# ETM-Code/eirgrid

Measured on AMD Instinct MI355X. Metric: 26-year episodes/sec, higher is better.
Workload: dtype f64

## Files before the change

eirgrid_amd/_native.py:

```python
from __future__ import annotations

import ctypes as C
import os

YEARS, N_ACTIONS, N_DEFICIT, N_COUNTS, N_TYPES = 26, 61, 15, 21, 15
GRID, CELLS, YEARLY_FIELDS = 51, 2601, 21
MAX_GENS, MAX_OFFSETS, RUN_CAP, DEF_CAP, ACT_CAP, ONCHIP_GENS = 4096, 4096, 4096, 4096, 4096, 512
TOPK_MAX = 64
STATS_LEN = 8 + 2 * YEARS * N_ACTIONS + YEARS * N_DEFICIT
CANDIDATE_BYTES = 8 + 8 + 32 + 4 * YEARS + 4 * YEARS + RUN_CAP + DEF_CAP
PACKET_BYTES = 8 * STATS_LEN + CANDIDATE_BYTES

EG_OK, EG_ERR_NO_DEVICE, EG_ERR_BAD_ARG, EG_ERR_HIP, EG_ERR_UNSUPPORTED, EG_ERR_NOMEM, EG_ERR_INTERNAL = 0, -1, -2, -3, -4, -5, -6
EG_EP_OK, EG_EP_OVERFLOW, EG_EP_NO_LOCATION, EG_EP_INTERNAL = 0, -1, -2, -3

LIB_PATH = os.environ.get("EIRGRID_LIB") or os.path.join(os.path.dirname(os.path.abspath(__file__)), "libeirgrid_hip.so")

_dp = C.POINTER(C.c_double)
_u8p = C.POINTER(C.c_uint8)
_u16p = C.POINTER(C.c_uint16)
_u32p = C.POINTER(C.c_uint32)
_i32p = C.POINTER(C.c_int32)
_u64p = C.POINTER(C.c_uint64)

# ... 20 lines not shown
class EgEpisodeOut(C.Structure):
    _fields_ = [("metrics", _dp), ("yearly", _dp), ("status", _i32p), ("n_run", _i32p), ("n_def", _i32p), ("n_act", _i32p),
                ("run_log", _u8p), ("def_log", _u8p), ("act_log", _u8p), ("n_gens", _i32p), ("gen_cell", _u16p),
                ("gen_pack", _u16p), ("n_offsets", _i32p), ("off_pack", _u16p), ("n_draws", _u64p), ("bytes_moved", _dp),
                ("n_chunks", _u32p)]


class EgPlanSet(C.Structure):
    _fields_ = [("n_plans", C.c_int32), ("best_count", _i32p), ("best_actions", _u8p), ("best_deficit_count", _i32p),
                ("best_deficit_actions", _u8p), ("best_actions_len", C.c_int64), ("best_deficit_actions_len", C.c_int64),
                ("names", C.POINTER(C.c_char_p))]


EXPORTS = [
    "eg_build_hash", "eg_last_error", "eg_device_count", "eg_create", "eg_destroy", "eg_rollout_batch", "eg_upload_snapshot",
    "eg_rollout_launch", "eg_rollout_launch_update", "eg_sync", "eg_last_batch_size", "eg_policy_hold", "eg_policy_rewind", "eg_replay_hoist", "eg_replay_hoist_stats", "eg_debug_hoist_stamps", "eg_fetch", "eg_timing_reset", "eg_timing_read", "eg_timing_read_grids", "eg_memory_report", "eg_update_stats", "eg_fetch_scores",
    "eg_fetch_episode_lists", "eg_fetch_record", "eg_fetch_best_run", "eg_best_result_track", "eg_fetch_best_result", "eg_evaluate_action_impact", "eg_place", "eg_find_suitable_location", "eg_debug_fill_lds", "eg_debug_occupy", "eg_policy_apply_reduced", "eg_policy_apply_packet", "eg_train_step",
    "eg_policy_push", "eg_device_rollout", "eg_device_apply", "eg_device_step", "eg_policy_pull",
    "eg_group_create", "eg_group_destroy", "eg_group_rank", "eg_group_push", "eg_group_step", "eg_group_pull", "eg_group_replay_hoist",
    "eg_group_best_result_track", "eg_group_fetch_best_result", "eg_top_k_track", "eg_fetch_top_k", "eg_rank_score",
    "eg_group_top_k_track", "eg_group_fetch_top_k", "eg_plans_validate", "eg_evaluate_plans", "eg_plans_load", "eg_plans_free",
    "eg_host_tables_create", "eg_host_tables_free", "eg_host_tables_f64", "eg_host_tables_i32",
    "eg_policy_new", "eg_policy_free", "eg_policy_snapshot_view", "eg_policy_get_tables", "eg_policy_set_tables",
    "eg_policy_get_scalar", "eg_policy_set_scalar", "eg_policy_get_list", "eg_policy_apply_episode", "eg_score_metrics",
    "eg_policy_save_json", "eg_policy_load_json", "eg_policy_append_weight_history", "eg_policy_export_improvement_csv", "eg_export_summary_csv", "eg_export_run_details",
]

_lib = None


def source_hash() -> str:
# ... 37 lines not shown
    L.eg_rollout_launch_update.restype = C.c_int32
    L.eg_rollout_launch_update.argtypes = [C.c_void_p, C.c_uint64, C.c_uint64, C.c_uint32, _u8p, C.c_void_p]
    L.eg_sync.restype = C.c_int32
    L.eg_sync.argtypes = [C.c_void_p]
    L.eg_last_batch_size.restype = C.c_uint32
    for f in (L.eg_policy_hold, L.eg_policy_rewind):
        f.restype = C.c_int32; f.argtypes = [C.c_void_p]
    L.eg_last_batch_size.argtypes = [C.c_void_p]
    if hasattr(L, "eg_replay_hoist") or not os.environ.get("EIRGRID_LIB"):
        L.eg_replay_hoist.restype = C.c_int32
        L.eg_replay_hoist.argtypes = [C.c_void_p, C.c_int32]
        L.eg_replay_hoist_stats.restype = C.c_int32
        L.eg_replay_hoist_stats.argtypes = [C.c_void_p, _u64p, _i32p]
        L.eg_debug_hoist_stamps.restype = C.c_int32
        L.eg_debug_hoist_stamps.argtypes = [C.c_void_p, _u64p]
    L.eg_fetch.restype = C.c_int32
    L.eg_fetch.argtypes = [C.c_void_p, C.POINTER(EgEpisodeOut)]
    L.eg_timing_reset.restype = C.c_int32
    L.eg_timing_reset.argtypes = [C.c_void_p]
    L.eg_timing_read.restype = C.c_int32
    L.eg_timing_read.argtypes = [C.c_void_p, _dp, _i32p]
    if hasattr(L, "eg_memory_report") or not os.environ.get("EIRGRID_LIB"):
        L.eg_memory_report.restype = C.c_int32
        L.eg_memory_report.argtypes = [C.c_void_p, _u64p, _u64p, _u64p]
    L.eg_timing_read_grids.restype = C.c_int32
    L.eg_timing_read_grids.argtypes = [C.c_void_p, _dp, _dp, _i32p]
    L.eg_update_stats.restype = C.c_int32
    L.eg_update_stats.argtypes = [C.c_void_p, C.c_void_p]
    L.eg_fetch_scores.restype = C.c_int32
    L.eg_fetch_scores.argtypes = [C.c_void_p, _dp]
# ... 123 lines not shown
```

eirgrid_amd/csrc/eg_api.cpp:

```cpp
#include <hip/hip_runtime.h>

#include <algorithm>
#include <cmath>
#include <cstring>
#include <map>
#include <mutex>
#include <cstdlib>
#include <string>
#include <vector>

#include "eg_internal.h"
#include "eg_policy_internal.h"
#define EG_RM static inline
#include "eg_reduced_math.h"

namespace eg {
namespace {
thread_local std::string g_error;
}
void set_error(const std::string& s) { g_error = s; }
}

using namespace eg;

// ... 56 lines not shown
  uint32_t push_iteration_count = 0;
  uint32_t push_failed = 0;
  uint32_t pulled_improvements = 0;
  uint8_t* d_packet = nullptr; uint8_t* h_packet = nullptr;
  uint32_t helper_max_episodes = 0;
  uint32_t heavy_slots_max = uint32_t((size_t(64) << 30) / (size_t(kRadiusClasses) * 2624 * sizeof(double)));
  uint32_t heavy_slots_wanted = 4096, launch_epoch = 0;
  bool heavy_slots_auto = true;
  bool hoist_on = false, hoist_supported = false;
  unsigned long long hoist_seq = 0;
  HoistInfo* d_hoist = nullptr; uint8_t* d_coop = nullptr;
  uint64_t hoist_batches = 0;
  int coop_force = 0;
  long long* d_stats_rep = nullptr;
  bool stats_rep_dirty = false;
  unsigned long long* d_solo = nullptr; uint32_t solo_cap = 0; unsigned long long solo_seq = 0;
  bool solo_on = true;
  uint8_t* d_eval_snap = nullptr;
  uint8_t* d_plans = nullptr; uint32_t plans_cap = 0;
  uint32_t* d_plan_index = nullptr; uint32_t plan_index_cap = 0;
};

namespace {

template <typename T>
void put(std::vector<uint8_t>& blob, size_t off, const std::vector<T>& v, size_t max_count) {
  const size_t n = v.size() < max_count ? v.size() : max_count;
  if (n) std::memcpy(blob.data() + off, v.data(), sizeof(T) * n);
}

void free_outputs(eg_ctx* c) {
// ... 25 lines not shown
        sum += ms;
      }
    for (int a = 0; a < 2; ++a)
      for (int b = 0; b < 2; ++b) {
        if (!(a ? lean : heavy) || !(b ? lean : heavy)) continue;
        EG_HIP(hipEventSynchronize(c->ev[i][2 * b + 1]));
        float ms = 0.f;
        EG_HIP(hipEventElapsedTime(&ms, c->ev[i][2 * a], c->ev[i][2 * b + 1]));
        if (ms > best) best = ms;
      }
    c->total_ms += double(best); c->grids_ms += double(sum); c->n_launches += 1; c->ring_pending -= 1;
  }
  return EG_OK;
}
int prepare_heavy(eg_ctx* c, uint32_t n_heavy, bool known_short) {
  constexpr size_t kSlotBytes = size_t(kRadiusClasses) * 2624 * sizeof(double), kTileBytes = size_t(kMaxVariants) * 64 * sizeof(double);
  if (known_short && !c->dev.heavy) n_heavy = 0;
  uint32_t want = c->heavy_slots_wanted;
  if (c->heavy_slots_auto && want > 0) {
    while (want < n_heavy && want < c->heavy_slots_max) want = want * 2u < c->heavy_slots_max ? want * 2u : c->heavy_slots_max;
  }
  if (want > 0 && n_heavy > 0 && (!c->dev.heavy || want > c->dev.heavy_slots)) {
    void* pool = nullptr;
    if (c->dev.heavy) {
      EG_HIP(hipDeviceSynchronize());
      for (auto it = c->allocs.begin(); it != c->allocs.end(); ++it) if (*it == c->dev.heavy) { c->allocs.erase(it); break; }
      (void)hipFree(c->dev.heavy);
      c->dev.heavy = nullptr; c->dev.heavy_slots = 0; c->dev.heavy_tiles = nullptr;
    }
    if (!c->dev.heavy_claim) {
      void* claim = nullptr;
      if (hipMalloc(&claim, 64) != hipSuccess) { (void)hipGetLastError(); c->heavy_slots_wanted = 0; want = 0; }
      else { EG_HIP(hipMemset(claim, 0xFF, 64)); c->allocs.push_back(claim); c->dev.heavy_claim = static_cast<unsigned*>(claim); }
    }
    while (want > 0 && hipMalloc(&pool, (kSlotBytes + kTileBytes) * want) != hipSuccess) {
      (void)hipGetLastError();
      pool = nullptr;
      want = want > 4096u ? want / 2u : 0u;
      c->heavy_slots_auto = false; c->heavy_slots_wanted = want;
    }
    if (pool) {
      c->allocs.push_back(pool); c->dev.heavy = static_cast<uint8_t*>(pool); c->dev.heavy_slots = want;
      c->dev.heavy_tiles = reinterpret_cast<double*>(static_cast<uint8_t*>(pool) + kSlotBytes * want);
    }
  }
  c->launch_epoch = (c->launch_epoch + 1u) & 0xFFFu;
  if (c->launch_epoch == 0xFFFu) c->launch_epoch = 0u;
  c->dev.heavy_epoch = c->launch_epoch;
  return EG_OK;
}
int topk_select(eg_ctx* c, uint32_t n, uint64_t first_index, int mode, bool use_score_list, const uint8_t* d_state, int k) {
  if (n > c->tk_cap) {
    if (c->d_tk_score) (void)hipFree(c->d_tk_score);
    if (c->d_tk_key) (void)hipFree(c->d_tk_key);
    if (c->d_tk_blocks) (void)hipFree(c->d_tk_blocks);
    c->d_tk_score = nullptr; c->d_tk_key = nullptr; c->d_tk_blocks = nullptr; c->tk_cap = 0;
    EG_HIP(hipMalloc((void**)&c->d_tk_score, sizeof(double) * n));
    EG_HIP(hipMalloc((void**)&c->d_tk_key, sizeof(unsigned long long) * n));
// ... 54 lines not shown
    if (plan.d_stats_rep != nullptr && c->stats_rep_dirty) {
      if (c->stream_heavy) EG_HIP(hipStreamSynchronize(c->stream_heavy));
      EG_HIP(hipMemsetAsync(c->d_stats_rep, 0, sizeof(long long) * size_t(kStatsReplicas) * EG_STATS_LEN, nullptr));
      c->stats_rep_dirty = false;
    }
  }
  if (plan.n_heavy > 0 && !plan.helper_waves && !plan.skip_long && !c->hoist_on) {
    if (c->solo_on) {
      if (plan.n_heavy > c->solo_cap) {
        if (c->d_solo) (void)hipFree(c->d_solo);
        c->d_solo = nullptr; c->solo_cap = 0;
        EG_HIP(hipMalloc((void**)&c->d_solo, sizeof(unsigned long long) * plan.n_heavy));
        EG_HIP(hipMemsetAsync(c->d_solo, 0, sizeof(unsigned long long) * plan.n_heavy, nullptr));
        c->solo_cap = plan.n_heavy;
      }
      plan.solo_seq = ++c->solo_seq; plan.d_solo = c->d_solo;
    }
  }
  if (c->hoist_on && plan.n_heavy > 0) {
    plan.hoist_seq = ++c->hoist_seq; plan.d_hoist = c->d_hoist; plan.coop_out = c->d_coop; plan.coop_force = c->coop_force;
    c->hoist_batches += 1;
  }
  if (split) {
    EG_HIP(hipEventRecord(c->ev_fork[slot], nullptr));
    EG_HIP(hipStreamWaitEvent(c->stream_heavy, c->ev_fork[slot], 0));
    if (list_long || plan.hoist_seq != 0ull) plan.go_event = c->ev_go[slot];
  }
  if (plan.d_stats_rep != nullptr) c->stats_rep_dirty = true;
  const int lr = launch_rollout(c->dev, c->snap, c->out, seed, first_index, n, d_mask, period, d_stats, plan);
  if (lr != 0) { set_error(std::string("k_rollout launch: ") + hipGetErrorString((hipError_t)lr)); return EG_ERR_HIP; }
  if (split) {
// ... 32 lines not shown
    if (rc != EG_OK) return rc;
    if (c->dev.heavy && chunk > c->dev.heavy_slots) chunk = c->dev.heavy_slots;
    RolloutPlan plan{};
    plan.plans = true; plan.helper_waves = helper;
    plan.n_short = first ? n_short : 0u;
    plan.n_heavy = plan.n_short + chunk; plan.n_lean = 0; plan.mode = 1u;
    plan.d_index = c->d_plan_index; plan.d_index_long = c->d_plan_index + n_short + done;
    if (chunk > 0 && !helper && c->solo_on) {
      if (chunk > c->solo_cap) {
        if (c->d_solo) (void)hipFree(c->d_solo);
        c->d_solo = nullptr; c->solo_cap = 0;
        EG_HIP(hipMalloc((void**)&c->d_solo, sizeof(unsigned long long) * chunk));
        EG_HIP(hipMemsetAsync(c->d_solo, 0, sizeof(unsigned long long) * chunk, nullptr));
        c->solo_cap = chunk;
      }
      plan.solo_seq = ++c->solo_seq; plan.d_solo = c->d_solo;
    }
    if (c->ring_pending == eg_ctx::kTimingRing) { rc = collect_timing(c, 1); if (rc != EG_OK) return rc; }
    const int slot = c->ring_head;
    for (int k = 0; k < 4; ++k) plan.ev[k] = c->ev[slot][k];
    const int lr = launch_rollout(c->dev, S, c->out, seed, first_index, n, nullptr, 1u, nullptr, plan);
    if (lr != 0) { set_error(std::string("k_rollout launch (plan batch): ") + hipGetErrorString((hipError_t)lr)); return EG_ERR_HIP; }
    c->ev_used[slot] = 1;
    c->ring_head = (c->ring_head + 1) % eg_ctx::kTimingRing; c->ring_pending += 1;
    done += chunk;
  }
  c->last_n = n; c->last_first = first_index;
  return EG_OK;
}

}
// ... 759 lines not shown
  EG_HIP(hipMemcpy(&word, c->d_hoist, sizeof(word), hipMemcpyDeviceToHost));
  if (batches_armed) *batches_armed = c->hoist_batches;
  static_assert(offsetof(HoistInfo, served_seq) == 0, "the served word comes first");
  if (last_batch_hoisted) *last_batch_hoisted = (c->hoist_seq != 0ull && word == c->hoist_seq) ? 1 : 0;
  return EG_OK;
}

int32_t eg_debug_hoist_stamps(eg_ctx* c, uint64_t stamps[8]) {
  if (!c || !stamps) return EG_ERR_BAD_ARG;
  EG_HIP(hipSetDevice(c->device));
  EG_HIP(hipDeviceSynchronize());
  EG_HIP(hipMemcpy(stamps, reinterpret_cast<const uint8_t*>(c->d_hoist) + offsetof(HoistInfo, stamps), 8 * sizeof(uint64_t), hipMemcpyDeviceToHost));
  return EG_OK;
}

int32_t eg_policy_hold(eg_ctx* c) {
  if (!c || !c->snap_valid) { set_error("eg_policy_hold: push a policy first"); return EG_ERR_BAD_ARG; }
  EG_HIP(hipSetDevice(c->device));
  if (!c->d_snap_held) EG_HIP(hipMalloc((void**)&c->d_snap_held, snap::total));
  EG_HIP(hipMemcpyAsync(c->d_snap_held, c->d_snap, snap::total, hipMemcpyDeviceToDevice, nullptr));
  c->long_list_hint_held = c->long_list_hint; c->list_exact_held = c->list_exact;
  return EG_OK;
}

int32_t eg_policy_rewind(eg_ctx* c) {
  if (!c || !c->d_snap_held) { set_error("eg_policy_rewind: nothing held"); return EG_ERR_BAD_ARG; }
  EG_HIP(hipSetDevice(c->device));
  const int lr = launch_rewind(c->d_snap, c->d_snap_held, c->d_list_len, nullptr);
  if (lr != 0) { set_error(std::string("k_rewind launch: ") + hipGetErrorString((hipError_t)lr)); return EG_ERR_HIP; }
  c->long_list_hint = c->long_list_hint_held; c->list_exact = c->list_exact_held;
// ... 447 lines not shown
```

eirgrid_amd/csrc/eg_internal.h:

```cpp
#pragma once
#include <cstddef>
#include <cstdint>
#include <string>
#include <vector>

#include "eirgrid_hip.h"

namespace eg {

constexpr int kYears = EG_YEARS;
constexpr int kTypes = EG_N_TYPES;
constexpr int kCells = EG_CELLS;
constexpr int kGrid = EG_GRID;
constexpr int kRadiusClasses = 6;
constexpr int kMaxReach = 12;
constexpr int kMults = 3;
constexpr int kOffsetTypes = 4;
constexpr int kPsStride = 2624;
constexpr int kDrCompact = 352;
constexpr int kLdsGens = EG_ONCHIP_GENS;
constexpr int kShortReplayMax = 96;
constexpr int kMaxVariants = 12;
constexpr int kTileW = 8;
constexpr int kTileCols = (kGrid + kTileW - 1) / kTileW;
// ... 76 lines not shown
constexpr size_t crank = a16(cbase + 8 * size_t(kYears) * kMaxVariants * kCells);
constexpr size_t ucell = a16(crank + 2 * size_t(kYears) * kMaxVariants * kCells);
constexpr size_t umax = a16(ucell + 8 * size_t(kMaxVariants) * kCells);
constexpr size_t rmax = a16(umax + 8 * size_t(kMaxVariants) * 64);
constexpr size_t total = a16(rmax + 8 * size_t(kYears) * kMaxVariants * 64);
}

struct DevTables {
  const uint8_t* base;
  double size_factor;
  int32_t n_existing;
  int32_t n_variants;
  uint32_t heavy_slots, heavy_epoch;
  uint8_t* heavy;
  unsigned* heavy_claim;
  double* heavy_tiles;
  uint32_t solo_tiles;
#define EG_TAB(name, type) EG_HD const type* name() const { return reinterpret_cast<const type*>(base + tab::name); }
  EG_TAB(usage, double) EG_TAB(population, double)
  EG_TAB(pre_co2, double) EG_TAB(pre_tg, double) EG_TAB(pre_ig, double) EG_TAB(pre_sg, double) EG_TAB(pre_optot, double)
  EG_TAB(inflation, double) EG_TAB(carbon_price, double) EG_TAB(out_mw, double) EG_TAB(co2_t, double)
  EG_TAB(pre_opcnt, int32_t) EG_TAB(variant, int32_t) EG_TAB(cls, int32_t) EG_TAB(rclass, int32_t) EG_TAB(marine, int32_t)
  EG_TAB(reach, int32_t)
  EG_TAB(dr, double) EG_TAB(m03, double) EG_TAB(t12, double) EG_TAB(offv, double) EG_TAB(offc, double) EG_TAB(cc, double)
  EG_TAB(ps, PsRec) EG_TAB(pbase, double) EG_TAB(pcell, uint32_t) EG_TAB(hv_lists, uint32_t) EG_TAB(hv_quads, int32_t) EG_TAB(dr_meta, int32_t) EG_TAB(dr_compact, double)
  EG_TAB(te_cell, double) EG_TAB(coastf, double) EG_TAB(cbase, double) EG_TAB(crank, uint16_t) EG_TAB(ucell, double) EG_TAB(umax, double) EG_TAB(rmax, double)
#undef EG_TAB
};

struct DevState {
  double learning_rate, exploration_rate;
// ... 202 lines not shown
```

eirgrid_amd/csrc/eg_replay_solo.h:

```cpp
#pragma once

namespace solo {

struct Lists {
  unsigned long long gen_pack;
  __device__ __forceinline__ static int* words() { return reinterpret_cast<int*>(sm.pol); }
  __device__ __forceinline__ int gpack_at(int i) const {
    __builtin_amdgcn_fence(__ATOMIC_RELEASE, "workgroup");
    return tail_u16(gen_pack, i);
  }
  __device__ __forceinline__ void gpack_put(int, int) const {}
  __device__ __forceinline__ void opack_put(int, int) const {}
  __device__ __forceinline__ int cls(int t) const { return (sm.type_info[t] >> 12) & 3; }
  __device__ __forceinline__ double out(int t) const { return sm.type_out[t]; }
  __device__ __forceinline__ void year_end(int yi, int ngen, int noff) const { words()[yi] = ngen; words()[EG_YEARS + yi] = noff; }
  __device__ __forceinline__ void finish(int run_pos, int def_pos, int act_pos, int ngen, int noff, unsigned long long bytes) const {
    int* w = words();
    w[52] = run_pos; w[53] = def_pos; w[54] = act_pos; w[55] = ngen; w[56] = noff;
    *reinterpret_cast<unsigned long long*>(w + 58) = bytes;
  }
};
static_assert(snap::kPolRow * 8 >= 60 * 4, "the script's lengths fit the policy row block");

constexpr int kEnt = 8;
struct Entries { int base[kEnt], delta[kEnt], dd[kEnt]; double fac[kEnt]; };
__device__ __forceinline__ void load_entries(Entries& E, int lane) {
#pragma unroll
  for (int k = 0; k < kEnt; ++k) {
    const uint32_t en = sh2.box[k * kWave + lane];
    const int rc = (int)(en >> 19), di = (int)(en & 31u) - 16, dj = (int)((en >> 5) & 31u) - 16;
    E.base[k] = rc * kFieldStride; E.delta[k] = di * kGrid + dj; E.dd[k] = (di & 0xFFFF) | (int)((unsigned)dj << 16);
    E.fac[k] = factor_by_q<false>(rc, (int)offsetof(Smem, dr), (int)((en >> 10) & 511u));
  }
}
template <int kN>
__device__ __forceinline__ void field_add(unsigned long long field_addr, const Entries& E, int cell) {
  const GlobalF64 base = (GlobalF64)field_addr;
  const int gi = cell / kGrid, gj = cell - gi * kGrid;
  double val[kN]; int off[kN];
#pragma unroll
  for (int k = 0; k < kN; ++k) {
    const int ci = gi + (int)(short)(E.dd[k] & 0xFFFF), cj = gj + (E.dd[k] >> 16);
    const bool inside = (unsigned)ci < (unsigned)kGrid && (unsigned)cj < (unsigned)kGrid;
    off[k] = E.base[k] + (inside ? cell + E.delta[k] : kCells);
// ... 35 lines not shown
  solo::Lists ls{(unsigned long long)O.gen_pack(e)};
  if (!rs::script(T, S, O, e, ls, lane)) return;
  __builtin_amdgcn_fence(__ATOMIC_RELEASE, "workgroup");
  wave_sync();
  EG_SS(1);
  const int* words = solo::Lists::words();
  const int n_gens = __builtin_amdgcn_readfirstlane(words[55]);

  Episode ep;
  ep.ngen = 0; ep.chunks = 0; ep.heavy = -1; ep.heavy_classes = 0; ep.heavy_quads = 0;
  uint16_t* gen_cell = O.gen_cell(e);
  const ListTail tail = {(unsigned long long)gen_cell, (unsigned long long)O.gen_pack(e), (unsigned long long)O.off_pack(e)};
  PrefixCache prefix_cache0 = {0.0, -1, 0};
  uint32_t search_seq = 0;
  int tile_variants = 0;
  int pk_block = 0;
  solo::Entries E;
#pragma unroll
  for (int k = 0; k < solo::kEnt; ++k) { E.base[k] = 0; E.delta[k] = 0; E.dd[k] = 0; E.fac[k] = 1.0; }
  for (int g = 0; g < n_gens; ++g) {
    if ((g & (kWave - 1)) == 0) pk_block = g + lane < n_gens ? tail_u16(tail.gen_pack, g + lane) : 0;
    const int pk = __builtin_amdgcn_readlane(pk_block, g & (kWave - 1));
    const int t = pk & 15, yi = (pk >> 4) & 31, m = pk >> 9;
    double m03v = 0.0;
    int cell = -1;
    bool placed = false;
    auto between = [] {};
    EG_SS(2);
    if (ep.ngen >= kHeavyGens && ep.heavy != -2) {
      const unsigned long long slot_bytes = (unsigned long long)(kRadiusClasses * kFieldStride) * 8ull;
      if (ep.heavy == -1) ep.heavy = heavy_claim(T, lane);
      if (ep.heavy >= 0) {
        const int info = __builtin_amdgcn_readfirstlane(sm.type_info[t]);
        const int hv = info & 15, hrc = (info >> 4) & 15;
        const unsigned long long class_addr = (unsigned long long)T.heavy + (unsigned long long)ep.heavy * slot_bytes + (unsigned long long)(hrc * kFieldStride) * 8ull;
        const unsigned long long tiles_addr = (unsigned long long)T.heavy_tiles + (unsigned long long)((ep.heavy * kMaxVariants + hv) * 64) * 8ull;
        if (!((ep.heavy_classes >> hrc) & 1)) {
          heavy_build_class<false>(class_addr, tail.gen_cell, lane, hrc, throughput_table(info), (info >> 8) & 15, ep.ngen);
          ep.heavy_classes |= 1 << hrc;
          ep.heavy_quads = __builtin_amdgcn_readfirstlane(T.hv_quads()[ep.heavy_classes]);
          wave_sync();
#pragma unroll
          for (int k = 0; k < kBoxLds / kWave; ++k) sh2.box[k * kWave + lane] = T.hv_lists()[ep.heavy_classes * 1024 + k * kWave + lane];
          wave_sync();
          solo::load_entries(E, lane);
        }
        int hr = kTilesUndecided;
        if (T.solo_tiles && !((tile_variants >> hv) & 1)) {
          ((GlobalF64)tiles_addr)[lane] = T.umax()[hv * 64 + lane];
          tile_variants |= 1 << hv;
        }
        if (T.solo_tiles) hr = place_tiles((unsigned long long)T.base, yi * kMaxVariants + hv, class_addr, tiles_addr, tail.gen_cell, T.size_factor, lane, hrc, throughput_table(info), ep.ngen);
        if (hr == kTilesUndecided) {
          const size_t yv = (size_t)(yi * kMaxVariants + hv) * kPsStride, yc = (size_t)(yi * kMaxVariants + hv) * kPcStride;
          hr = place_heavy<false>((unsigned long long)(T.ps() + yv), (unsigned long long)(T.pbase() + yc), (unsigned long long)(T.pcell() + yc), class_addr,
                                  tail.gen_cell, T.size_factor, lane, hrc, throughput_table(info), ep.ngen);
        }
        if (hr >= 0) { cell = hr & 0xFFFF; ep.chunks += hr >> 16; placed = true; }
      }
    }
    if (!placed && ep.ngen > kLdsGens) {
      const int info = __builtin_amdgcn_readfirstlane(sm.type_info[t]);
      const int xr = place_exact_long<false>((unsigned long long)(T.ps() + (size_t)(yi * kMaxVariants + (info & 15)) * kPsStride), tail.gen_cell,
                                             T.size_factor, lane, (info >> 4) & 15, throughput_table(info), ep.ngen);
      cell = xr < 0 ? -1 : (xr & 0xFFFF);
      if (xr >= 0) ep.chunks += xr >> 16;
      placed = true;
// ... 77 lines not shown
```

eirgrid_amd/csrc/eg_rollout.hip:

```cpp
#include <hip/hip_runtime.h>
#include <cstddef>
#include <hip/hip_ext.h>

#include "eg_internal.h"

#define EG_DETPOW_QUAL __device__ __forceinline__
#include "eg_detpow.h"
#define EG_RM __device__ __forceinline__
#include "eg_reduced_math.h"

namespace eg {
namespace {

constexpr int kWave = 64;
constexpr int kD2Max = 144, kD2Stride = 146;
constexpr int kCmdYear = 1 << 30;
constexpr int kHelperWaves = 1;
constexpr int kSpinCap = 1 << 20;
constexpr int kSearchLost = -2;
constexpr double kMinWeight = 0.0001;
constexpr double kMaxWeight = 0.999;
constexpr double kMaxCost = 50000000000.0;
constexpr int kBattery = 12, kPeaker = 8;
constexpr int kNothing = 60, kFirstOffset = 45, kFirstOther = 57;
// ... 1049 lines not shown
  wave_sync();
#ifdef EG_STAMPS
  asm volatile("s_waitcnt vmcnt(0)" ::: "memory");
  const unsigned long long ts2 = __builtin_readcyclecounter();
#endif
  const ChunkBest b = heavy_exact<kLatency>(list_addr, tail_cells, size_factor, lane, rc, tbl, ngen_s, ncand, ncand == 1 && solo >= 0 ? __builtin_amdgcn_readlane(lcell, solo) : -1);
  if (!(b.score > 0.0)) return kSearchFallback;
#ifdef EG_STAMPS
  if (lane == 0) { sm.hdbg[0][0] += ts1 - ts0; sm.hdbg[0][1] += ts2 - ts1; sm.hdbg[0][2] += __builtin_readcyclecounter() - ts2; sm.hdbg[1][0] += (unsigned long long)K; sm.hdbg[1][1] += (unsigned long long)ncand; sm.hdbg[1][2] += 1ull; }
#endif
  return heavy_result(b, lane, K, ncand);
}

constexpr int kTilesUndecided = -4;
static_assert(kTileW * kTileW == kWave, "a cell of a tile per lane");
__device__ __noinline__ int place_tiles(unsigned long long tab_addr, int yv, unsigned long long class_addr, unsigned long long tiles_addr,
                                        unsigned long long tail_cells, double size_factor, int lane, int rc, int tbl, int ngen) {
#ifdef EG_STAMPS
  const unsigned long long ts0 = __builtin_readcyclecounter();
#endif
  asm volatile("s_waitcnt vmcnt(0)" ::: "memory");
  const int ngen_s = __builtin_amdgcn_readfirstlane(ngen);
  constexpr int kChunks = (kCells + kWave - 1) / kWave, kGroup = 4, kGroups = (kChunks + kGroup - 1) / kGroup;
  constexpr double kKeep = 1.0 - 0x1p-30, kKeepTile = 1.0 - 0x1p-29;
  constexpr int kNoTile = 63;
  static_assert(kNoTile >= kTiles && (kNoTile / kTileCols) * kTileW >= kGrid, "kNoTile is off the grid");
  auto uniform_u64 = [](unsigned long long a) { return ((unsigned long long)(unsigned)__builtin_amdgcn_readfirstlane((int)(a >> 32)) << 32) | (unsigned)__builtin_amdgcn_readfirstlane((int)a); };
  const unsigned long long tab_s = uniform_u64(tab_addr), a_s = uniform_u64(class_addr), t_s = uniform_u64(tiles_addr);
  const unsigned long long yv_s = (unsigned long long)(unsigned)__builtin_amdgcn_readfirstlane(yv);
  const unsigned long long cb_s = tab_s + tab::cbase + yv_s * (8ull * kCells), rk_s = tab_s + tab::crank + yv_s * (2ull * kCells);
  const unsigned long long pb_s = tab_s + tab::pbase + yv_s * (8ull * kPcStride), rm_s = tab_s + tab::rmax + yv_s * (8ull * 64);
  const unsigned long long uc_s = tab_s + tab::ucell + (yv_s % kMaxVariants) * (8ull * kCells);
  const GlobalF64 gmax = (GlobalF64)t_s;
  auto field_at = [&](int cell) { return __hip_atomic_load((GlobalF64)(a_s + (unsigned long long)((unsigned)cell * 8u)), __ATOMIC_RELAXED, __HIP_MEMORY_SCOPE_AGENT); };
  auto cb_at = [&](int cell) { return *(GlobalF64c)(cb_s + (unsigned long long)((unsigned)cell * 8u)); };
  auto uc_at = [&](int cell) { return *(GlobalF64c)(uc_s + (unsigned long long)((unsigned)cell * 8u)); };
  auto rk_at = [&](int cell) { return (int)*(const uint16_t __attribute__((address_space(1)))*)(rk_s + (unsigned long long)((unsigned)cell * 2u)); };
  const double gb = lane >= 1 && lane < kGroups ? *(GlobalF64c)(pb_s + (unsigned long long)((unsigned)(lane * kGroup * kWave) * 8u)) : 0.0;
  const double bound = lane < kTiles ? *(GlobalF64c)(rm_s + (unsigned long long)((unsigned)lane * 8u)) * field_load(gmax + lane) : 0.0;
  unsigned long long left = __ballot(bound > 0.0);
  if (left == 0ull) return kSearchFallback;
  const unsigned hb = (unsigned)__double2hiint(bound);
  const unsigned h1 = wave_max_u32(hb);
  int ta = __ffsll((long long)(left & __ballot(hb == h1))) - 1, tb = kNoTile;
  {
    const unsigned long long rest = left & ~(1ull << ta);
    const unsigned h2 = wave_max_u32(lane == ta ? 0u : hb);
    const unsigned long long second = rest & __ballot(hb == h2);
    if (rest != 0ull) tb = __ffsll((long long)(second != 0ull ? second : rest)) - 1;
  }
  double lm = 0.0, l2 = 0.0;
  int lrank = 0, lcell = -1;
#ifdef EG_STAMPS
  int tiles = 0;
#endif
  auto fold = [&](double v, int r, int c) {
    const double key = __hiloint2double(__double2hiint(v), (__double2loint(v) & ~63) | (r >> 6));
    const bool larger = key > lm;
    l2 = vmax64(l2, vmin64(lm, key));
    lm = vmax64(lm, key);
    lrank = larger ? r : lrank; lcell = larger ? c : lcell;
  };
#pragma nounroll
  for (;;) {
    left &= ~(1ull << ta) & ~(1ull << tb);
    const int ia = (ta / kTileCols) * kTileW + (lane >> 3), ja = (ta % kTileCols) * kTileW + (lane & 7);
    const int ib = (tb / kTileCols) * kTileW + (lane >> 3), jb = (tb % kTileCols) * kTileW + (lane & 7);
    const bool ina = ia < kGrid && ja < kGrid, inb = ib < kGrid && jb < kGrid;
    const int ca = ina ? ia * kGrid + ja : 0, cb = inb ? ib * kGrid + jb : 0;
    const double fa = field_at(ca), fb = field_at(cb), pa = cb_at(ca), pb = cb_at(cb), ua = uc_at(ca), ub = uc_at(cb);
    const int ra = rk_at(ca), rb = rk_at(cb);
    fold(ina ? pa * fa : 0.0, ra, ca);
    fold(inb ? pb * fb : 0.0, rb, cb);
    const unsigned gha = wave_max_u32(ina ? (unsigned)__double2hiint(ua * fa) : 0u), ghb = wave_max_u32(inb ? (unsigned)__double2hiint(ub * fb) : 0u);
    if (lane == 0) {
      gmax[ta] = __hiloint2double((int)gha, -1);
      if (tb < kTiles) gmax[tb] = __hiloint2double((int)ghb, -1);
    }
#ifdef EG_STAMPS
    tiles += tb < kTiles ? 2 : 1;
#endif
    const double m_lo = __hiloint2double((int)wave_max_u32((unsigned)__double2hiint(lm)), 0);
    left &= __ballot(bound >= m_lo * kKeepTile);
    if (left == 0ull) break;
    ta = __ffsll((long long)left) - 1;
    const unsigned long long rest = left & (left - 1ull);
    tb = rest != 0ull ? __ffsll((long long)rest) - 1 : kNoTile;
  }
  const double M = wave_max_f64(lm);
  if (!(M >= 1e-250)) return kSearchFallback;
#ifdef EG_STAMPS
  const unsigned long long ts1 = __builtin_readcyclecounter();
// ... 1605 lines not shown
```

eirgrid_amd/engine.py:

```python
from __future__ import annotations

import ctypes as C
from dataclasses import dataclass, fields

import numpy as np

from . import _native as N
from .world import World

BASE_YEAR, END_YEAR = 2025, 2050

YEARLY_COLUMNS = [
    "year", "total_population", "total_power_usage", "total_power_generation", "power_balance",
    "average_public_opinion", "yearly_capital_cost", "total_capital_cost", "inflation_factor", "total_co2_emissions",
    "total_carbon_offset", "net_co2_emissions", "yearly_carbon_credit_revenue", "total_carbon_credit_revenue",
    "yearly_energy_sales_revenue", "total_energy_sales_revenue", "active_generators", "yearly_upgrade_costs",
    "yearly_closure_costs", "yearly_total_cost", "total_cost",
]


def _p(a, t):
    return a.ctypes.data_as(C.POINTER(t))


# ... 394 lines not shown

    def hold(self):
        N.check(N.lib().eg_policy_hold(self.h), "eg_policy_hold")

    def rewind(self):
        N.check(N.lib().eg_policy_rewind(self.h), "eg_policy_rewind")

    def replay_hoist(self, on: bool = True) -> None:
        N.check(N.lib().eg_replay_hoist(self.h, int(bool(on))), "eg_replay_hoist")

    def replay_hoist_stats(self):
        n, last = C.c_uint64(), C.c_int32()
        N.check(N.lib().eg_replay_hoist_stats(self.h, C.byref(n), C.byref(last)), "eg_replay_hoist_stats")
        return int(n.value), bool(last.value)

    def pull(self, weights: ActionWeights):
        N.check(N.lib().eg_policy_pull(self.h, weights.h), "eg_policy_pull")

    def sync(self):
        N.check(N.lib().eg_sync(self.h), "eg_sync")

    def fetch(self, n_episodes: int = None) -> BatchResult:
        last = int(N.lib().eg_last_batch_size(self.h))
        if n_episodes is not None and n_episodes != last:
            raise ValueError(f"fetch({n_episodes}): the last launched batch holds {last} episodes")
        res = BatchResult.alloc(last)
        out = res.struct()
        N.check(N.lib().eg_fetch(self.h, C.byref(out)), "eg_fetch")
        return res

# ... 154 lines not shown
```

include/eirgrid_hip.h:

```cpp
#ifndef EIRGRID_HIP_H
#define EIRGRID_HIP_H

#include <stdint.h>

#ifdef __cplusplus
extern "C" {
#endif

#define EG_YEARS 26
#define EG_N_ACTIONS 61
#define EG_N_DEFICIT 15
#define EG_N_COUNTS 21
#define EG_N_TYPES 15
#define EG_GRID 51
#define EG_CELLS (EG_GRID * EG_GRID)
#define EG_YEARLY_FIELDS 21

#define EG_MAX_GENS 4096
#define EG_MAX_OFFSETS 4096
#define EG_RUN_CAP 4096
#define EG_DEF_CAP 4096
#define EG_ACT_CAP 4096
#define EG_ONCHIP_GENS 512

// ... 178 lines not shown
                               uint64_t noise_seed);
int32_t eg_train_step(eg_ctx *, eg_policy *, const eg_opts *opts, uint64_t seed, uint64_t first_episode_index,
                      uint32_t n_episodes, const uint8_t *replay_mask , uint64_t noise_seed);
int32_t eg_policy_push(eg_ctx *, const eg_policy *, const eg_opts *opts);
int32_t eg_device_rollout(eg_ctx *, uint64_t seed, uint64_t first_episode_index, uint32_t n_episodes, uint32_t replay_period,
                          void *d_packet);
int32_t eg_device_apply(eg_ctx *, const void *d_packets, int32_t n_packets, void *d_own_packet, uint64_t noise_seed);
int32_t eg_device_step(eg_ctx *, uint64_t seed, uint64_t first_episode_index, uint32_t n_episodes, uint32_t replay_period,
                       uint64_t noise_seed);
int32_t eg_policy_pull(eg_ctx *, eg_policy *);
int32_t eg_policy_hold(eg_ctx *);
int32_t eg_policy_rewind(eg_ctx *);
int32_t eg_replay_hoist(eg_ctx *, int32_t on);
int32_t eg_replay_hoist_stats(eg_ctx *, uint64_t *batches_armed, int32_t *last_batch_hoisted);
int32_t eg_debug_hoist_stamps(eg_ctx *, uint64_t stamps[8]);
int32_t eg_policy_save_json(const eg_policy *, const char *path);
eg_policy *eg_policy_load_json(const char *path);
int32_t eg_policy_append_weight_history(const eg_policy *, const char *path, uint64_t iteration);
int32_t eg_policy_export_improvement_csv(const eg_policy *, const char *path);
int32_t eg_export_summary_csv(const eg_episode_out *run, const char *path, const char *timestamp);
int32_t eg_export_run_details(const eg_world *world, const char *const *settlement_names, const eg_episode_out *run,
                              const char *out_dir, uint64_t offset_seed);
double eg_score_metrics(const double metrics[4], int32_t cost_only);

#ifdef __cplusplus
}
#endif
#endif
```

Measured before the change: 8.676 million.

## Keep solo tile bounds and row tables in LDS instead of global memory

The per-variant tile maxima used by the solo placement path move out of a global heavy_tiles pool into LDS words, reusing the box and opack regions and storing only the high 32 bits. The rmax and pbase rows are staged into a shared row once per year/variant, and entry lists are read straight from the global hv_lists table rather than copied through LDS. A debug export for counting solo-served episodes is also added. The aim is fewer global round trips and a smaller heavy allocation, with the risk of LDS aliasing against other users of box/opack and lower-precision stored bounds.

```diff
diff --git a/eirgrid_amd/_native.py b/eirgrid_amd/_native.py
--- a/eirgrid_amd/_native.py
+++ b/eirgrid_amd/_native.py
@@ -58,7 +58,7 @@
 
 EXPORTS = [
     "eg_build_hash", "eg_last_error", "eg_device_count", "eg_create", "eg_destroy", "eg_rollout_batch", "eg_upload_snapshot",
-    "eg_rollout_launch", "eg_rollout_launch_update", "eg_sync", "eg_last_batch_size", "eg_policy_hold", "eg_policy_rewind", "eg_replay_hoist", "eg_replay_hoist_stats", "eg_debug_hoist_stamps", "eg_fetch", "eg_timing_reset", "eg_timing_read", "eg_timing_read_grids", "eg_memory_report", "eg_update_stats", "eg_fetch_scores",
+    "eg_rollout_launch", "eg_rollout_launch_update", "eg_sync", "eg_last_batch_size", "eg_policy_hold", "eg_policy_rewind", "eg_replay_hoist", "eg_replay_hoist_stats", "eg_debug_hoist_stamps", "eg_debug_solo_served", "eg_fetch", "eg_timing_reset", "eg_timing_read", "eg_timing_read_grids", "eg_memory_report", "eg_update_stats", "eg_fetch_scores",
     "eg_fetch_episode_lists", "eg_fetch_record", "eg_fetch_best_run", "eg_best_result_track", "eg_fetch_best_result", "eg_evaluate_action_impact", "eg_place", "eg_find_suitable_location", "eg_debug_fill_lds", "eg_debug_occupy", "eg_policy_apply_reduced", "eg_policy_apply_packet", "eg_train_step",
     "eg_policy_push", "eg_device_rollout", "eg_device_apply", "eg_device_step", "eg_policy_pull",
     "eg_group_create", "eg_group_destroy", "eg_group_rank", "eg_group_push", "eg_group_step", "eg_group_pull", "eg_group_replay_hoist",
@@ -126,6 +126,9 @@
         L.eg_replay_hoist_stats.argtypes = [C.c_void_p, _u64p, _i32p]
         L.eg_debug_hoist_stamps.restype = C.c_int32
         L.eg_debug_hoist_stamps.argtypes = [C.c_void_p, _u64p]
+    if hasattr(L, "eg_debug_solo_served") or not os.environ.get("EIRGRID_LIB"):
+        L.eg_debug_solo_served.restype = C.c_int32
+        L.eg_debug_solo_served.argtypes = [C.c_void_p, C.POINTER(C.c_uint32), C.POINTER(C.c_uint32)]
     L.eg_fetch.restype = C.c_int32
     L.eg_fetch.argtypes = [C.c_void_p, C.POINTER(EgEpisodeOut)]
     L.eg_timing_reset.restype = C.c_int32
diff --git a/eirgrid_amd/csrc/eg_api.cpp b/eirgrid_amd/csrc/eg_api.cpp
--- a/eirgrid_amd/csrc/eg_api.cpp
+++ b/eirgrid_amd/csrc/eg_api.cpp
@@ -94,7 +94,7 @@
   int coop_force = 0;
   long long* d_stats_rep = nullptr;
   bool stats_rep_dirty = false;
-  unsigned long long* d_solo = nullptr; uint32_t solo_cap = 0; unsigned long long solo_seq = 0;
+  unsigned long long* d_solo = nullptr; uint32_t solo_cap = 0; unsigned long long solo_seq = 0; uint32_t solo_last_n = 0;
   bool solo_on = true;
   uint8_t* d_eval_snap = nullptr;
   uint8_t* d_plans = nullptr; uint32_t plans_cap = 0;
@@ -150,7 +150,7 @@
   return EG_OK;
 }
 int prepare_heavy(eg_ctx* c, uint32_t n_heavy, bool known_short) {
-  constexpr size_t kSlotBytes = size_t(kRadiusClasses) * 2624 * sizeof(double), kTileBytes = size_t(kMaxVariants) * 64 * sizeof(double);
+  constexpr size_t kSlotBytes = size_t(kRadiusClasses) * 2624 * sizeof(double);
   if (known_short && !c->dev.heavy) n_heavy = 0;
   uint32_t want = c->heavy_slots_wanted;
   if (c->heavy_slots_auto && want > 0) {
@@ -162,14 +162,14 @@
       EG_HIP(hipDeviceSynchronize());
       for (auto it = c->allocs.begin(); it != c->allocs.end(); ++it) if (*it == c->dev.heavy) { c->allocs.erase(it); break; }
       (void)hipFree(c->dev.heavy);
-      c->dev.heavy = nullptr; c->dev.heavy_slots = 0; c->dev.heavy_tiles = nullptr;
+      c->dev.heavy = nullptr; c->dev.heavy_slots = 0;
     }
     if (!c->dev.heavy_claim) {
       void* claim = nullptr;
       if (hipMalloc(&claim, 64) != hipSuccess) { (void)hipGetLastError(); c->heavy_slots_wanted = 0; want = 0; }
       else { EG_HIP(hipMemset(claim, 0xFF, 64)); c->allocs.push_back(claim); c->dev.heavy_claim = static_cast<unsigned*>(claim); }
     }
-    while (want > 0 && hipMalloc(&pool, (kSlotBytes + kTileBytes) * want) != hipSuccess) {
+    while (want > 0 && hipMalloc(&pool, kSlotBytes * want) != hipSuccess) {
       (void)hipGetLastError();
       pool = nullptr;
       want = want > 4096u ? want / 2u : 0u;
@@ -177,7 +177,6 @@
     }
     if (pool) {
       c->allocs.push_back(pool); c->dev.heavy = static_cast<uint8_t*>(pool); c->dev.heavy_slots = want;
-      c->dev.heavy_tiles = reinterpret_cast<double*>(static_cast<uint8_t*>(pool) + kSlotBytes * want);
     }
   }
   c->launch_epoch = (c->launch_epoch + 1u) & 0xFFFu;
@@ -262,7 +261,7 @@
         EG_HIP(hipMemsetAsync(c->d_solo, 0, sizeof(unsigned long long) * plan.n_heavy, nullptr));
         c->solo_cap = plan.n_heavy;
       }
-      plan.solo_seq = ++c->solo_seq; plan.d_solo = c->d_solo;
+      plan.solo_seq = ++c->solo_seq; plan.d_solo = c->d_solo; c->solo_last_n = plan.n_heavy;
     }
   }
   if (c->hoist_on && plan.n_heavy > 0) {
@@ -325,7 +324,7 @@
         EG_HIP(hipMemsetAsync(c->d_solo, 0, sizeof(unsigned long long) * chunk, nullptr));
         c->solo_cap = chunk;
       }
-      plan.solo_seq = ++c->solo_seq; plan.d_solo = c->d_solo;
+      plan.solo_seq = ++c->solo_seq; plan.d_solo = c->d_solo; c->solo_last_n = chunk;
     }
     if (c->ring_pending == eg_ctx::kTimingRing) { rc = collect_timing(c, 1); if (rc != EG_OK) return rc; }
     const int slot = c->ring_head;
@@ -1115,6 +1114,19 @@
   return EG_OK;
 }
 
+int32_t eg_debug_solo_served(eg_ctx* c, uint32_t* launched, uint32_t* served) {
+  if (!c || !launched || !served) return EG_ERR_BAD_ARG;
+  EG_HIP(hipSetDevice(c->device));
+  EG_HIP(hipDeviceSynchronize());
+  *launched = 0; *served = 0;
+  if (!c->d_solo || c->solo_seq == 0ull || c->solo_last_n == 0u) return EG_OK;
+  std::vector<unsigned long long> words(c->solo_last_n);
+  EG_HIP(hipMemcpy(words.data(), c->d_solo, sizeof(unsigned long long) * words.size(), hipMemcpyDeviceToHost));
+  *launched = c->solo_last_n;
+  for (unsigned long long w : words) *served += w == c->solo_seq ? 1u : 0u;
+  return EG_OK;
+}
+
 int32_t eg_policy_hold(eg_ctx* c) {
   if (!c || !c->snap_valid) { set_error("eg_policy_hold: push a policy first"); return EG_ERR_BAD_ARG; }
   EG_HIP(hipSetDevice(c->device));
diff --git a/eirgrid_amd/csrc/eg_internal.h b/eirgrid_amd/csrc/eg_internal.h
--- a/eirgrid_amd/csrc/eg_internal.h
+++ b/eirgrid_amd/csrc/eg_internal.h
@@ -114,7 +114,6 @@
   uint32_t heavy_slots, heavy_epoch;
   uint8_t* heavy;
   unsigned* heavy_claim;
-  double* heavy_tiles;
   uint32_t solo_tiles;
 #define EG_TAB(name, type) EG_HD const type* name() const { return reinterpret_cast<const type*>(base + tab::name); }
   EG_TAB(usage, double) EG_TAB(population, double)
diff --git a/eirgrid_amd/csrc/eg_replay_solo.h b/eirgrid_amd/csrc/eg_replay_solo.h
--- a/eirgrid_amd/csrc/eg_replay_solo.h
+++ b/eirgrid_amd/csrc/eg_replay_solo.h
@@ -24,10 +24,10 @@
 
 constexpr int kEnt = 8;
 struct Entries { int base[kEnt], delta[kEnt], dd[kEnt]; double fac[kEnt]; };
-__device__ __forceinline__ void load_entries(Entries& E, int lane) {
+__device__ __forceinline__ void load_entries(Entries& E, const uint32_t* list, int lane) {
 #pragma unroll
   for (int k = 0; k < kEnt; ++k) {
-    const uint32_t en = sh2.box[k * kWave + lane];
+    const uint32_t en = list[k * kWave + lane];
     const int rc = (int)(en >> 19), di = (int)(en & 31u) - 16, dj = (int)((en >> 5) & 31u) - 16;
     E.base[k] = rc * kFieldStride; E.delta[k] = di * kGrid + dj; E.dd[k] = (di & 0xFFFF) | (int)((unsigned)dj << 16);
     E.fac[k] = factor_by_q<false>(rc, (int)offsetof(Smem, dr), (int)((en >> 10) & 511u));
@@ -93,6 +93,7 @@
   PrefixCache prefix_cache0 = {0.0, -1, 0};
   uint32_t search_seq = 0;
   int tile_variants = 0;
+  int tile_yv = -1;
   int pk_block = 0;
   solo::Entries E;
 #pragma unroll
@@ -113,23 +114,30 @@
         const int info = __builtin_amdgcn_readfirstlane(sm.type_info[t]);
         const int hv = info & 15, hrc = (info >> 4) & 15;
         const unsigned long long class_addr = (unsigned long long)T.heavy + (unsigned long long)ep.heavy * slot_bytes + (unsigned long long)(hrc * kFieldStride) * 8ull;
-        const unsigned long long tiles_addr = (unsigned long long)T.heavy_tiles + (unsigned long long)((ep.heavy * kMaxVariants + hv) * 64) * 8ull;
         if (!((ep.heavy_classes >> hrc) & 1)) {
           heavy_build_class<false>(class_addr, tail.gen_cell, lane, hrc, throughput_table(info), (info >> 8) & 15, ep.ngen);
           ep.heavy_classes |= 1 << hrc;
           ep.heavy_quads = __builtin_amdgcn_readfirstlane(T.hv_quads()[ep.heavy_classes]);
-          wave_sync();
-#pragma unroll
-          for (int k = 0; k < kBoxLds / kWave; ++k) sh2.box[k * kWave + lane] = T.hv_lists()[ep.heavy_classes * 1024 + k * kWave + lane];
-          wave_sync();
-          solo::load_entries(E, lane);
+          solo::load_entries(E, T.hv_lists() + ep.heavy_classes * 1024, lane);
         }
         int hr = kTilesUndecided;
         if (T.solo_tiles && !((tile_variants >> hv) & 1)) {
-          ((GlobalF64)tiles_addr)[lane] = T.umax()[hv * 64 + lane];
+          if (lane < kTiles) tile_words(hv)[lane] = (uint32_t)__double2hiint(T.umax()[hv * 64 + lane]);
           tile_variants |= 1 << hv;
         }
-        if (T.solo_tiles) hr = place_tiles((unsigned long long)T.base, yi * kMaxVariants + hv, class_addr, tiles_addr, tail.gen_cell, T.size_factor, lane, hrc, throughput_table(info), ep.ngen);
+        if (T.solo_tiles) {
+          const int yv = yi * kMaxVariants + hv;
+          if (yv != tile_yv) {
+            int ln = lane;
+            asm volatile("" : "+v"(ln));
+            const double rm = ln < kTiles ? T.rmax()[yv * 64 + ln] : 0.0;
+            const double gb = ln >= 1 && ln < kTileGroups ? T.pbase()[(size_t)yv * kPcStride + ln * 4 * kWave] : 0.0;
+            tile_row()[ln] = rm;
+            if (ln < kTileGroups) tile_row()[kWave + ln] = gb;
+            tile_yv = yv;
+          }
+          hr = place_tiles((unsigned long long)T.base, yv, class_addr, hv, tail.gen_cell, T.size_factor, lane, hrc, throughput_table(info), ep.ngen);
+        }
         if (hr == kTilesUndecided) {
           const size_t yv = (size_t)(yi * kMaxVariants + hv) * kPsStride, yc = (size_t)(yi * kMaxVariants + hv) * kPcStride;
           hr = place_heavy<false>((unsigned long long)(T.ps() + yv), (unsigned long long)(T.pbase() + yc), (unsigned long long)(T.pcell() + yc), class_addr,
diff --git a/eirgrid_amd/csrc/eg_rollout.hip b/eirgrid_amd/csrc/eg_rollout.hip
--- a/eirgrid_amd/csrc/eg_rollout.hip
+++ b/eirgrid_amd/csrc/eg_rollout.hip
@@ -1087,30 +1087,38 @@
 
 constexpr int kTilesUndecided = -4;
 static_assert(kTileW * kTileW == kWave, "a cell of a tile per lane");
-__device__ __noinline__ int place_tiles(unsigned long long tab_addr, int yv, unsigned long long class_addr, unsigned long long tiles_addr,
+constexpr int kTileGroups = ((kCells + kWave - 1) / kWave + 3) / 4;
+constexpr int kBoxVariants = kBoxLds / kTiles;
+static_assert((kMaxVariants - kBoxVariants) * kTiles * 4 <= (int)sizeof(Smem::opack) && offsetof(Smem, opack) % 4 == 0, "the tile bounds of every variant fit");
+__device__ __forceinline__ uint32_t* tile_words(int variant) {
+  return variant < kBoxVariants ? sh2.box + variant * kTiles : reinterpret_cast<uint32_t*>(sm.opack) + (variant - kBoxVariants) * kTiles;
+}
+constexpr int kTileRow = 32;
+static_assert(kTileRow * 8 >= 60 * 4 && kTileRow + kWave + kTileGroups <= snap::kPolRow, "the row fits between the script's lengths and the block's end");
+__device__ __forceinline__ double* tile_row() { return sm.pol + kTileRow; }
+__device__ __noinline__ int place_tiles(unsigned long long tab_addr, int yv, unsigned long long class_addr, int variant,
                                         unsigned long long tail_cells, double size_factor, int lane, int rc, int tbl, int ngen) {
 #ifdef EG_STAMPS
   const unsigned long long ts0 = __builtin_readcyclecounter();
 #endif
-  asm volatile("s_waitcnt vmcnt(0)" ::: "memory");
   const int ngen_s = __builtin_amdgcn_readfirstlane(ngen);
-  constexpr int kChunks = (kCells + kWave - 1) / kWave, kGroup = 4, kGroups = (kChunks + kGroup - 1) / kGroup;
+  constexpr int kChunks = (kCells + kWave - 1) / kWave, kGroup = 4, kGroups = kTileGroups;
   constexpr double kKeep = 1.0 - 0x1p-30, kKeepTile = 1.0 - 0x1p-29;
   constexpr int kNoTile = 63;
   static_assert(kNoTile >= kTiles && (kNoTile / kTileCols) * kTileW >= kGrid, "kNoTile is off the grid");
   auto uniform_u64 = [](unsigned long long a) { return ((unsigned long long)(unsigned)__builtin_amdgcn_readfirstlane((int)(a >> 32)) << 32) | (unsigned)__builtin_amdgcn_readfirstlane((int)a); };
-  const unsigned long long tab_s = uniform_u64(tab_addr), a_s = uniform_u64(class_addr), t_s = uniform_u64(tiles_addr);
+  const unsigned long long tab_s = uniform_u64(tab_addr), a_s = uniform_u64(class_addr);
   const unsigned long long yv_s = (unsigned long long)(unsigned)__builtin_amdgcn_readfirstlane(yv);
   const unsigned long long cb_s = tab_s + tab::cbase + yv_s * (8ull * kCells), rk_s = tab_s + tab::crank + yv_s * (2ull * kCells);
-  const unsigned long long pb_s = tab_s + tab::pbase + yv_s * (8ull * kPcStride), rm_s = tab_s + tab::rmax + yv_s * (8ull * 64);
   const unsigned long long uc_s = tab_s + tab::ucell + (yv_s % kMaxVariants) * (8ull * kCells);
-  const GlobalF64 gmax = (GlobalF64)t_s;
+  uint32_t* const gw = tile_words(__builtin_amdgcn_readfirstlane(variant));
   auto field_at = [&](int cell) { return __hip_atomic_load((GlobalF64)(a_s + (unsigned long long)((unsigned)cell * 8u)), __ATOMIC_RELAXED, __HIP_MEMORY_SCOPE_AGENT); };
   auto cb_at = [&](int cell) { return *(GlobalF64c)(cb_s + (unsigned long long)((unsigned)cell * 8u)); };
   auto uc_at = [&](int cell) { return *(GlobalF64c)(uc_s + (unsigned long long)((unsigned)cell * 8u)); };
   auto rk_at = [&](int cell) { return (int)*(const uint16_t __attribute__((address_space(1)))*)(rk_s + (unsigned long long)((unsigned)cell * 2u)); };
-  const double gb = lane >= 1 && lane < kGroups ? *(GlobalF64c)(pb_s + (unsigned long long)((unsigned)(lane * kGroup * kWave) * 8u)) : 0.0;
-  const double bound = lane < kTiles ? *(GlobalF64c)(rm_s + (unsigned long long)((unsigned)lane * 8u)) * field_load(gmax + lane) : 0.0;
+  wave_sync();
+  const double gb = lane < kTileGroups ? tile_row()[kWave + lane] : 0.0;
+  const double bound = lane < kTiles ? tile_row()[lane] * __hiloint2double((int)gw[lane], -1) : 0.0;
   unsigned long long left = __ballot(bound > 0.0);
   if (left == 0ull) return kSearchFallback;
   const unsigned hb = (unsigned)__double2hiint(bound);
@@ -1141,14 +1149,15 @@
     const int ib = (tb / kTileCols) * kTileW + (lane >> 3), jb = (tb % kTileCols) * kTileW + (lane & 7);
     const bool ina = ia < kGrid && ja < kGrid, inb = ib < kGrid && jb < kGrid;
     const int ca = ina ? ia * kGrid + ja : 0, cb = inb ? ib * kGrid + jb : 0;
+    asm volatile("s_waitcnt vmcnt(0)" ::: "memory");
     const double fa = field_at(ca), fb = field_at(cb), pa = cb_at(ca), pb = cb_at(cb), ua = uc_at(ca), ub = uc_at(cb);
     const int ra = rk_at(ca), rb = rk_at(cb);
     fold(ina ? pa * fa : 0.0, ra, ca);
     fold(inb ? pb * fb : 0.0, rb, cb);
     const unsigned gha = wave_max_u32(ina ? (unsigned)__double2hiint(ua * fa) : 0u), ghb = wave_max_u32(inb ? (unsigned)__double2hiint(ub * fb) : 0u);
     if (lane == 0) {
-      gmax[ta] = __hiloint2double((int)gha, -1);
-      if (tb < kTiles) gmax[tb] = __hiloint2double((int)ghb, -1);
+      gw[ta] = gha;
+      if (tb < kTiles) gw[tb] = ghb;
     }
 #ifdef EG_STAMPS
     tiles += tb < kTiles ? 2 : 1;
diff --git a/eirgrid_amd/engine.py b/eirgrid_amd/engine.py
--- a/eirgrid_amd/engine.py
+++ b/eirgrid_amd/engine.py
@@ -432,6 +432,11 @@
         N.check(N.lib().eg_replay_hoist_stats(self.h, C.byref(n), C.byref(last)), "eg_replay_hoist_stats")
         return int(n.value), bool(last.value)
 
+    def solo_served(self):
+        n, served = C.c_uint32(), C.c_uint32()
+        N.check(N.lib().eg_debug_solo_served(self.h, C.byref(n), C.byref(served)), "eg_debug_solo_served")
+        return int(n.value), int(served.value)
+
     def pull(self, weights: ActionWeights):
         N.check(N.lib().eg_policy_pull(self.h, weights.h), "eg_policy_pull")
 
diff --git a/include/eirgrid_hip.h b/include/eirgrid_hip.h
--- a/include/eirgrid_hip.h
+++ b/include/eirgrid_hip.h
@@ -216,6 +216,7 @@
 int32_t eg_replay_hoist(eg_ctx *, int32_t on);
 int32_t eg_replay_hoist_stats(eg_ctx *, uint64_t *batches_armed, int32_t *last_batch_hoisted);
 int32_t eg_debug_hoist_stamps(eg_ctx *, uint64_t stamps[8]);
+int32_t eg_debug_solo_served(eg_ctx *, uint32_t *launched, uint32_t *served);
 int32_t eg_policy_save_json(const eg_policy *, const char *path);
 eg_policy *eg_policy_load_json(const char *path);
 int32_t eg_policy_append_weight_history(const eg_policy *, const char *path, uint64_t iteration);
```

Result: no change. 8.690 million (median of 6 runs) (+0.2%).
